# ferdean/lsa-fw

Measured on AMD Instinct MI355X. Metric: converged eigenpairs/sec (k=20, shift-invert), higher is better.
Workload: dtype c128

## Files before the change

### lsa-fw_amd/csrc/ndlu.hip

```cpp
#include "ndlu_internal.h"

namespace {

void nd_free(lsa_ndlu* f) {
    if (!f) return;
    ndlu_multi_free(f);
    for (void* p : {f->d_top, (void*)f->d_top_icmap, (void*)f->d_top_jobs, (void*)f->d_top_tiles})
        if (p) (void)hipFree(p);
    for (void* p : {(void*)f->d_lnodes_bwd, (void*)f->d_dist_nodes, (void*)f->d_child_ptr, (void*)f->d_child_idx, f->d_xstage, f->d_xg, (void*)f->d_tgoff, f->d_tg})
        if (p) (void)hipFree(p);
    for (void* p : {(void*)f->d_nodes, (void*)f->d_lnodes, (void*)f->d_gell, (void*)f->d_idx, (void*)f->d_cmap, (void*)f->d_tiles,
                    (void*)f->d_chunk_nodes, (void*)f->d_asm_dst, (void*)f->d_asm_src, (void*)f->d_ipiv, (void*)f->d_rowq, (void*)f->d_flag, (void*)f->d_xflag, (void*)f->d_maxabs,
                    f->d_lfac, f->d_ufac, f->d_work, f->d_upd, f->d_ubuf, f->d_xb, f->d_acc, f->d_tmp, f->d_ybuf, (void*)f->d_cand[0], (void*)f->d_cand[1], f->d_dinv})
        if (p) (void)hipFree(p);
    if (f->ev_panel) (void)hipEventDestroy(f->ev_panel);
    if (f->ev_pivots) (void)hipEventDestroy(f->ev_pivots);
    if (f->side) (void)hipStreamDestroy(f->side);
    delete f;
}

int nd_setup_top(lsa_ctx* ctx, lsa_ndlu* f, const std::vector<NdNodeDev>& nodes) {
    const NdSymbolic& S = f->S;
    f->top = NdTop{};
    f->top_level = -1;
// ... 56 lines not shown
    f->top_tiles[0] = (int32_t)tiles.size() / 2;
    for (int32_t ci = 0; ci < K; ++ci)
        for (int32_t di = 0; di < K; ++di) {
            const NdNodeDev &nc = nodes[(size_t)S.child_idx[(size_t)c0 + ci]], &nd = nodes[(size_t)S.child_idx[(size_t)c0 + di]];
            add(NdTopJob{tp.node[ci].off * s + oR, nd.lfac_off + (int64_t)nd.m * nd.m, tp.node[ci].off * s + tp.node[di].off, ci == di ? nc.lfac_off : -1, nc.m,
                         nd.m, nd.f - nd.m, (int32_t)s, nd.m, nc.m, 2, 1, nd.cmap_off, 0});
        }
    f->top_tiles[1] = (int32_t)tiles.size() / 2 - f->top_tiles[0];
    LSA_CHECK(upload(ctx, icmap, &f->d_top_icmap));
    LSA_CHECK(upload(ctx, jobs, &f->d_top_jobs));
    LSA_CHECK(upload(ctx, tiles, &f->d_top_tiles));
    LSA_HIP_ALLOC(ctx, hipMalloc(&f->d_top, (size_t)(s * s) * esize(f->dtype)));
    f->top = tp;
    f->top_level = lr;
    f->top_replaced_entries = replaced;
    f->solve_launches -= 2;
    return LSA_OK;
}


struct TileBuffer {
    std::vector<int32_t> tiles;
    void begin(TileList& tl) {
        tl.off = (int64_t)tiles.size() / 2;
        tl.count = 0;
    }
    void push(TileList& tl, int32_t a, int32_t b) {
        tiles.push_back(a);
        tiles.push_back(b);
        ++tl.count;
    }
};

void nd_setup_knobs(lsa_ndlu* f) {
    const char* e = getenv("LSA_ND_TP_MIN");
    f->tp_min = e && *e ? std::max(1, atoi(e)) : 512;
    const char* sbm = getenv("LSA_ND_SB_MIN");
    f->sb_min = std::max(f->tp_min, sbm && *sbm ? std::max(1, atoi(sbm)) : 1024);
    f->ycap = kNB;
    const char* sbc = getenv("LSA_ND_SB_COLS");
    f->sb_cols = sbc && *sbc ? std::min(1024, std::max(kGT, atoi(sbc) / kGT * kGT)) : kSB;
}

bool nd_setup_ordered(const NdSymbolic& S) {
    const bool dist = S.nranks > 1;
    bool ordered = true;
    for (size_t k = 0; k < S.perm.size() && ordered; ++k) ordered = S.perm[k] == (int32_t)k || dist;
    if (dist)
        for (int32_t t = 0; t < S.nt && ordered; ++t)
            for (int32_t r = 1; r < S.m[(size_t)t]; ++r)
                if (S.idx[(size_t)S.idx_off[(size_t)t] + r] != S.idx[(size_t)S.idx_off[(size_t)t]] + r) {
                    ordered = false;
                    break;
                }
    return ordered;
}

int64_t nd_setup_budget(const NdSymbolic& S, size_t es, int64_t free_agreed) {
    size_t free_b = 0, total_b = 0;
    if (hipMemGetInfo(&free_b, &total_b) != hipSuccess) free_b = (size_t)16 << 30;
    const int64_t after = (int64_t)free_b - S.factor_entries * (int64_t)es;
    int64_t budget = std::max<int64_t>(after / 4, (int64_t)256 << 20) / (int64_t)es;
    if (S.has_dist) budget = std::max<int64_t>((free_agreed > 0 ? free_agreed : (int64_t)free_b) / 6, (int64_t)256 << 20) / (int64_t)es;
    if (const char* e = getenv("LSA_ND_WORK_MB")) budget = std::max<int64_t>(atoll(e), 1) * (1 << 20) / (int64_t)es;
    return budget;
}

std::vector<NdNodeDev> nd_setup_nodes(const NdSymbolic& S, const NdMemoryPlan& P) {
    std::vector<NdNodeDev> nodes((size_t)S.nt);
    for (int32_t t = 0; t < S.nt; ++t) {
        NdNodeDev& nd = nodes[(size_t)t];
// ... 95 lines not shown
        for (int32_t rb = r0; rb < r1; rb += sh)
            for (int32_t cb = 0; cb < TN; cb += sw)
                for (int32_t r = rb; r < std::min(rb + sh, r1); ++r)
                    for (int32_t cc = cb; cc < std::min(cb + sw, TN); ++cc) seq[x].push_back((r << 16) | cc);
    }
    size_t pos[8] = {0, 0, 0, 0, 0, 0, 0, 0};
    for (int64_t left = (int64_t)TM * TN; left > 0; --left) {
        int x = (int)(tl.count % 8);
        for (int tries = 0; tries < 8 && pos[x] >= seq[x].size(); ++tries) x = (x + 1) % 8;
        tb.push(tl, t, seq[x][pos[x]++]);
    }
}

void nd_setup_chunk_tiles(const NdSymbolic& S, NdChunk& c, TileBuffer& tb) {
    auto node = [&](int32_t q) { return S.lvl_nodes[(size_t)c.node_begin + q]; };
    int32_t lvl_children = 0;
    for (int32_t q = 0; q < c.node_count; ++q) lvl_children = std::max(lvl_children, S.child_ptr[(size_t)node(q) + 1] - S.child_ptr[(size_t)node(q)]);
    c.ext.assign((size_t)lvl_children, TileList());
    for (int32_t r = 0; r < lvl_children; ++r) {
        tb.begin(c.ext[(size_t)r]);
        for (int32_t q = 0; q < c.node_count; ++q) {
            const int32_t t = node(q);
            if (S.child_ptr[(size_t)t] + r >= S.child_ptr[(size_t)t + 1]) continue;
            const int32_t ch = S.child_idx[(size_t)S.child_ptr[(size_t)t] + r];
            if (S.kind[(size_t)t] == 4 && S.kind[(size_t)ch] != 2) continue;
            const int32_t bc = S.f[(size_t)ch] - S.m[(size_t)ch];
            for (int32_t i0 = 0; i0 < bc; i0 += 16) tb.push(c.ext[(size_t)r], ch, i0);
        }
    }
    tb.begin(c.unperm);
    for (int32_t q = 0; q < c.node_count; ++q)
        for (int32_t r0 = 0; r0 < S.m[(size_t)node(q)]; r0 += 16) tb.push(c.unperm, node(q), r0);
    static const bool xcd_order = !(getenv("LSA_ND_XCD_ORDER") && atoi(getenv("LSA_ND_XCD_ORDER")) == 0);
    for (int kind = 0; kind < 3; ++kind) {
        tb.begin(c.gemm[kind]);
        for (int32_t q = 0; q < c.node_count; ++q) {
            const int32_t t = node(q);
            const int32_t m = S.m[(size_t)t], b = S.f[(size_t)t] - m;
            if (b == 0) continue;
            const int32_t M = kind == 2 ? S.orows[(size_t)t] : S.brow[(size_t)t], N = kind == 0 ? m : b;
            if (M == 0) continue;
            const int32_t TM = (M + kGT - 1) / kGT, TN = (N + kGT - 1) / kGT;
            if ((int64_t)TM * TN >= 512 && xcd_order) {
                nd_push_xcd_order(tb, c.gemm[kind], t, TM, TN);
                continue;
            }
            for (int32_t tm = 0; tm < TM; ++tm)
                for (int32_t tn = 0; tn < TN; ++tn) tb.push(c.gemm[kind], t, (tm << 16) | tn);
        }
    }
    tb.begin(c.save);
    for (int32_t q = 0; q < c.node_count; ++q) {
        const int32_t t = node(q);
        for (int32_t r0 = 0; r0 < S.brow[(size_t)t]; r0 += 16) tb.push(c.save, t, r0);
    }
}

void nd_setup_chunk_xsteps(const NdSymbolic& S, const NdMemoryPlan& P, NdChunk& c) {
    std::vector<std::vector<NdChunk::XPiece>> queue((size_t)S.nranks);
    for (int32_t q = 0; q < c.node_count; ++q) {
        const int32_t t = S.lvl_nodes[(size_t)c.node_begin + q];
        if (S.kind[(size_t)t] != 4) continue;
        for (int32_t cp = S.child_ptr[(size_t)t]; cp < S.child_ptr[(size_t)t + 1]; ++cp) {
            const int32_t ch = S.child_idx[(size_t)cp];
            if (S.kind[(size_t)ch] == 2) continue;
            const int32_t bc = S.f[(size_t)ch] - S.m[(size_t)ch];
            if (bc == 0) continue;
// ... 250 lines not shown
    if (!ctx || !f || !C) return lsa_set_error(ctx, LSA_ERR_ARG, "lsa_ndlu_refactor: null argument");
    if (C->n != f->S.n || C->n != C->ncols || C->nnz != f->S.nnz || C->dtype != f->dtype)
        return lsa_set_error(ctx, LSA_ERR_ARG, "lsa_ndlu_refactor: the matrix does not match the analysed pattern");
    const double t0 = now_s();
    const int rc = ndlu_numeric(ctx, f, C);
    f->seconds_numeric = now_s() - t0;
    return rc;
}

static uint64_t mat_pattern_hash(const lsa_mat* P) {
    if (!P->h_hash) P->h_hash = std::make_shared<uint64_t>(0);
    if (*P->h_hash == 0) {
        const uint64_t h = nd_pattern_hash(P->n, P->h_rp.data(), P->h_ci.data());
        *P->h_hash = h ? h : 1;
    }
    return *P->h_hash;
}

static int nd_symbolic_phase(lsa_ctx* ctx, const lsa_mat* P, int dtype, int32_t leaf_size, const int8_t* constraint, bool strict,
                             lsa_ndlu** out) {
    *out = nullptr;
    if (P->n != P->ncols || P->row0 != 0) return lsa_set_error(ctx, LSA_ERR_ARG, "lsa_ndlu: needs a square, unsharded matrix");
    if ((int64_t)P->h_rp.size() != (int64_t)P->n + 1) return lsa_set_error(ctx, LSA_ERR_ARG, "lsa_ndlu: the matrix has no host copy of its pattern");
    if (leaf_size <= 0) leaf_size = nd_default_leaf(P->n);
    const double t0 = now_s();
    if (ctx->nd_cache) {
        lsa_ndlu* c = ctx->nd_cache;
        const uint64_t want = strict && constraint ? nd_constraint_hash(P->n, constraint) : 0;
        if (c->S.n == P->n && c->S.nnz == P->nnz && c->dtype == dtype && c->S.nranks == 1 && (c->S.tree_hash != 0 || c->S.leaf_size == leaf_size) &&
            (!strict || c->S.constraint_hash == want) &&
            c->S.pattern_hash == mat_pattern_hash(P)) {
            ctx->nd_cache = nullptr;
            c->seconds_analyse = 0.0;
            *out = c;
            return LSA_OK;
        }
        lsa_ndlu_drop_cache(ctx);
    }
    return nd_new_analysed(ctx, dtype, "lsa_ndlu", t0, 0, out, [&](NdSymbolic* S, char* err, int errlen) {
        return nd_analyse(P->n, P->h_rp.data(), P->h_ci.data(), leaf_size, constraint, S, err, errlen);
    });
}

int lsa_ndlu_prepare(lsa_ctx* ctx, const lsa_mat* P, int dtype, int32_t leaf_size, const int8_t* constraint) {
    if (!ctx || !P || (dtype != LSA_F64 && dtype != LSA_C128)) return lsa_set_error(ctx, LSA_ERR_ARG, "lsa_ndlu_prepare: bad argument");
    lsa_ndlu* f = nullptr;
    LSA_CHECK(nd_symbolic_phase(ctx, P, dtype, leaf_size, constraint, true, &f));
    lsa_ndlu_drop_cache(ctx);
    ctx->nd_cache = f;
    return LSA_OK;
}

int lsa_ndlu_prepare_tree(lsa_ctx* ctx, const lsa_mat* P, int dtype, int32_t ntree, const int32_t* first, const int32_t* size, const int32_t* parent) {
    if (!ctx || !P || (dtype != LSA_F64 && dtype != LSA_C128) || ntree < 0 || (ntree > 0 && (!first || !size || !parent)))
        return lsa_set_error(ctx, LSA_ERR_ARG, "lsa_ndlu_prepare_tree: bad argument");
    if (P->n != P->ncols || P->row0 != 0) return lsa_set_error(ctx, LSA_ERR_ARG, "lsa_ndlu_prepare_tree: needs a square, unsharded matrix");
    if ((int64_t)P->h_rp.size() != (int64_t)P->n + 1) return lsa_set_error(ctx, LSA_ERR_ARG, "lsa_ndlu_prepare_tree: the matrix has no host copy of its pattern");
    const double t0 = now_s();
    lsa_ndlu_drop_cache(ctx);
    lsa_ndlu* f = nullptr;
    LSA_CHECK(nd_new_analysed(ctx, dtype, "lsa_ndlu_prepare_tree", t0, 0, &f, [&](NdSymbolic* S, char* err, int errlen) {
        return nd_analyse_tree(P->n, P->h_rp.data(), P->h_ci.data(), ntree, first, size, parent, nullptr, 0, 1, S, err, errlen);
    }));
    ctx->nd_cache = f;
    return LSA_OK;
}
// ... 24 lines not shown
        return rc;
    }
    *out = f;
    return LSA_OK;
}

int lsa_ndlu_create_tree(lsa_ctx* ctx, const lsa_mat* C, int32_t ntree, const int32_t* first, const int32_t* size, const int32_t* parent,
                         const int32_t* owner, lsa_ndlu** out) {
    if (!ctx || !C || !out || ntree < 0) return lsa_set_error(ctx, LSA_ERR_ARG, "lsa_ndlu_create_tree: bad argument");
    *out = nullptr;
    if (C->n != C->ncols || C->row0 != 0) return lsa_set_error(ctx, LSA_ERR_ARG, "lsa_ndlu_create_tree: needs the whole square matrix (every rank holds it)");
    if ((int64_t)C->h_rp.size() != (int64_t)C->n + 1) return lsa_set_error(ctx, LSA_ERR_ARG, "lsa_ndlu_create_tree: the matrix has no host copy of its pattern");
    const double t0 = now_s();
    lsa_ndlu* f = nullptr;
    int setup_rc = LSA_OK;
    int64_t free_agreed = 0;
    if (ctx->nranks > 1) {
        size_t free_b = 0, total_b = 0;
        if (hipMemGetInfo(&free_b, &total_b) != hipSuccess) free_b = (size_t)16 << 30;
        if (ctx->nd_cache) {
            const lsa_ndlu* c = ctx->nd_cache;
            free_b += (size_t)(c->lfac_entries + c->ufac_entries + c->work_entries + c->upd_entries) * esize(c->dtype);
        }
        free_agreed = (int64_t)free_b;
        LSA_CHECK(k_agree_min_i64(ctx, &free_agreed));
    }
    if (ctx->nd_cache) {
        lsa_ndlu* c = ctx->nd_cache;
        if (c->S.tree_hash == nd_tree_hash(ntree, first, size, parent, owner, ctx->rank, ctx->nranks) && c->S.n == C->n && c->S.nnz == C->nnz && c->dtype == C->dtype &&
            c->S.pattern_hash == mat_pattern_hash(C)) {
            f = c;
            ctx->nd_cache = nullptr;
            f->seconds_analyse = 0.0;
        } else {
            lsa_ndlu_drop_cache(ctx);
        }
    }
    if (!f)
        setup_rc = nd_new_analysed(ctx, C->dtype, "lsa_ndlu_create_tree", t0, free_agreed, &f, [&](NdSymbolic* S, char* err, int errlen) {
            return nd_analyse_tree(C->n, C->h_rp.data(), C->h_ci.data(), ntree, first, size, parent, owner, ctx->rank, ctx->nranks, S, err, errlen);
        });
    setup_rc = k_agree_status(ctx, setup_rc);
    if (setup_rc != LSA_OK) {
        nd_free(f);
        return setup_rc;
    }
    const int rc = lsa_ndlu_refactor(ctx, f, C);
    if (rc != LSA_OK) {
        nd_free(f);
        return rc;
    }
    *out = f;
    return LSA_OK;
}

void lsa_ndlu_destroy(lsa_ndlu* f) {
    if (!f) return;
    lsa_ctx* ctx = f->ctx;
    if (ctx && ctx->stream) (void)hipStreamSynchronize(ctx->stream);
    if (ctx && !getenv("LSA_ND_NO_CACHE")) {
        lsa_ndlu_drop_cache(ctx);
        ctx->nd_cache = f;
        return;
    }
    nd_free(f);
}
// ... 193 lines not shown
```

### lsa-fw_amd/csrc/ndlu_factor.hip

```cpp
#include "ndlu_internal.h"

namespace {

template <typename T>
__global__ __launch_bounds__(256) void nd_maxabs2_kernel(int64_t nnz, const T* __restrict__ v, unsigned long long* __restrict__ out) {
    __shared__ double wmax[4];
    double best = 0.0;
    const int64_t stride = (int64_t)gridDim.x * blockDim.x;
    for (int64_t i = (int64_t)blockIdx.x * blockDim.x + threadIdx.x; i < nnz; i += stride) {
        const double a = s_abs2(v[i]);
        if (a == a && a > best) best = a;
        else if (a != a) best = a;
    }
    for (int o = 32; o > 0; o >>= 1) {
        const double other = __shfl_xor(best, o);
        best = (best != best) ? best : (other != other) ? other : fmax(best, other);
    }
    if ((threadIdx.x & 63) == 0) wmax[threadIdx.x >> 6] = best;
    __syncthreads();
    if (threadIdx.x == 0) {
        for (int w = 1; w < 4; ++w) best = (best != best) ? best : (wmax[w] != wmax[w]) ? wmax[w] : fmax(best, wmax[w]);
        atomicMax(out, (unsigned long long)__double_as_longlong(best));
    }
}
// ... 308 lines not shown
        const int32_t gc = col0 + qb;
        Ys[jb][qb] = (jb < nb && gc < m) ? yb[(size_t)jb * m + gc] : scalar_traits<T>::zero();
    }
    __syncthreads();
    T acc[4][4];
#pragma unroll
    for (int i = 0; i < 4; ++i)
#pragma unroll
        for (int j = 0; j < 4; ++j) acc[i][j] = scalar_traits<T>::zero();
    for (int k = 0; k < nb; ++k) {
        T av[4], bv[4];
#pragma unroll
        for (int i = 0; i < 4; ++i) av[i] = Ws[k][ty * 4 + i];
#pragma unroll
        for (int j = 0; j < 4; ++j) bv[j] = Ys[k][tx + 16 * j];
#pragma unroll
        for (int i = 0; i < 4; ++i)
#pragma unroll
            for (int j = 0; j < 4; ++j) fma_acc(acc[i][j], av[i], bv[j]);
    }
#pragma unroll
    for (int i = 0; i < 4; ++i) {
        const int32_t gr = row0 + ty * 4 + i;
        if (gr >= m) continue;
        const int32_t q = rq[gr];
        const bool is_piv = q >= kb && q < kb + nb;
#pragma unroll
        for (int j = 0; j < 4; ++j) {
            const int32_t gc = col0 + tx + 16 * j;
            if (gc >= m || (gc >= kb && gc < kb + nb)) continue;
            if ((gc >= skip_lo && gc < skip_hi) || (only_hi > only_lo && (gc < only_lo || gc >= only_hi))) continue;
            T* cptr = a + (size_t)gr * ld + gc;
            *cptr = is_piv ? acc[i][j] : s_add(*cptr, acc[i][j]);
        }
    }
}

constexpr int kTA = 8;

template <typename T>
struct tp_first {
    static constexpr int RPT = sizeof(T) == 16 ? 1 : 2;
    static constexpr int rows = 256 * RPT;
};

__host__ __device__ inline int32_t tp_sets(int32_t m, int32_t first_rows, int32_t round) {
    int32_t n = (m + first_rows - 1) / first_rows;
    for (int32_t r = 0; r < round; ++r) n = (n + kTA - 1) / kTA;
    return n;
}

template <typename T, bool FIRST, bool LAST>
__global__ __launch_bounds__(256) void nd_tp_round_kernel(const int32_t* __restrict__ lvl_nodes, const NdNodeDev* __restrict__ nodes,
                                                          const T* __restrict__ front, int32_t* __restrict__ ipiv, int32_t* __restrict__ rowq, int32_t kb,
                                                          int32_t round, const int32_t* __restrict__ cand_in, int32_t* __restrict__ cand_out,
                                                          T* __restrict__ dinv, int32_t* __restrict__ flag, double tiny2) {
    constexpr int RPT = FIRST ? tp_first<T>::RPT : 1;
    __shared__ unsigned long long skey[2];
    __shared__ T prow_s[2][kNB];
    __shared__ int32_t sel_s[kNB];
    __shared__ T Ds[LAST ? kNB : 1][kNB + 1];
    const int32_t t = lvl_nodes[blockIdx.x];
    const NdNodeDev nd = nodes[t];
    const int32_t m = nd.m, ld = nd.f;
    const int32_t w = min(kNB, m - kb);
    if (w <= 0) return;
// ... 233 lines not shown
                sm.Bs[p][(e >> 6) * LDBS + (e & 63)] = plane_of(pb[s], p);
            }
        }
        __syncthreads();
        if (kk + BK < K) gload(kk + BK);
#pragma unroll
        for (int k4 = 0; k4 < BK; k4 += 4) {
            if (kk + k4 >= K) break;
            double a[NPL][2], bb[NPL][2];
#pragma unroll
            for (int p = 0; p < NPL; ++p)
#pragma unroll
                for (int i = 0; i < 2; ++i) {
                    a[p][i] = sm.As[p][(wr + 16 * i + l15) * LDAS + k4 + l4];
                    bb[p][i] = sm.Bs[p][(k4 + l4) * LDBS + wc + 16 * i + l15];
                }
#pragma unroll
            for (int i = 0; i < 2; ++i)
#pragma unroll
                for (int j = 0; j < 2; ++j) {
                    acc[0][i][j] = __builtin_amdgcn_mfma_f64_16x16x4f64(a[0][i], bb[0][j], acc[0][i][j], 0, 0, 0);
                    if constexpr (NPL == 2) {
                        acc[0][i][j] = __builtin_amdgcn_mfma_f64_16x16x4f64(-a[NPL - 1][i], bb[NPL - 1][j], acc[0][i][j], 0, 0, 0);
                        acc[NPL - 1][i][j] = __builtin_amdgcn_mfma_f64_16x16x4f64(a[0][i], bb[NPL - 1][j], acc[NPL - 1][i][j], 0, 0, 0);
                        acc[NPL - 1][i][j] = __builtin_amdgcn_mfma_f64_16x16x4f64(a[NPL - 1][i], bb[0][j], acc[NPL - 1][i][j], 0, 0, 0);
                    }
                }
        }
        __syncthreads();
    }
}

template <typename T, int KIND>
__global__ __launch_bounds__(256) void nd_gemm_mfma_kernel(const int32_t* __restrict__ tiles, const NdNodeDev* __restrict__ nodes,
                                                           T* __restrict__ front, T* __restrict__ lfac, T* __restrict__ ufac) {
    constexpr int NPL = MfmaTile<T>::NPL;
    __shared__ MfmaTile<T> sm;
    const int32_t t = tiles[2 * blockIdx.x], packed = tiles[2 * blockIdx.x + 1];
    const int32_t tm = packed >> 16, tn = packed & 0xFFFF;
    const NdNodeDev nd = nodes[t];
    const int32_t m = nd.m, f = nd.f, b = f - m;
    T* F = front + nd.front_off;
    T* inv = nd.inv_off < 0 ? lfac + nd.lfac_off : front + nd.inv_off;
    T* invrows = lfac + nd.lfac_off;
    T* S1 = invrows + (size_t)nd.orows * m;
    T* S2 = ufac + nd.ufac_off;
    const T *A, *B;
    T* C;
    int32_t M, N, K, lda, ldb, ldc;
    if (KIND == 0) {
        A = F + (size_t)m * f, lda = f, B = inv, ldb = m, C = S1, ldc = m, M = nd.brow, N = m, K = m;
    } else if (KIND == 1) {
        A = S1, lda = m, B = F + m, ldb = f, C = F + (size_t)m * f + m, ldc = f, M = nd.brow, N = b, K = m;
    } else {
        A = invrows, lda = m, B = F + m, ldb = f, C = S2, ldc = b, M = nd.orows, N = b, K = m;
    }
    const int32_t row0 = tm * kGT, col0 = tn * kGT;
    mfma_d4 acc[NPL][2][2];
    mfma_tile_product<T>(
        K,
        [&](int r, int32_t k) {
            const int32_t gr = row0 + r;
            return (gr < M && k < K) ? A[(size_t)gr * lda + k] : scalar_traits<T>::zero();
        },
        [&](int32_t k, int c) {
            const int32_t gc = col0 + c;
            return (k < K && gc < N) ? B[(size_t)k * ldb + gc] : scalar_traits<T>::zero();
        },
        sm, acc);
    const int lane = threadIdx.x & 63, wave = threadIdx.x >> 6;
    const int wr = 32 * (wave >> 1), wc = 32 * (wave & 1), l15 = lane & 15, l4 = lane >> 4;
#pragma unroll
    for (int i = 0; i < 2; ++i)
#pragma unroll
        for (int r = 0; r < 4; ++r) {
            const int32_t gr = row0 + wr + 16 * i + l4 + 4 * r;
            if (gr >= M) continue;
#pragma unroll
            for (int j = 0; j < 2; ++j) {
                const int32_t gc = col0 + wc + 16 * j + l15;
                if (gc >= N) continue;
                T v;
                s_from(v, acc[0][i][j][r], acc[NPL - 1][i][j][r]);
                T* c = C + (size_t)gr * ldc + gc;
                if (KIND == 0) *c = s_sub(scalar_traits<T>::zero(), v);
                else if (KIND == 1) *c = s_add(*c, v);
                else *c = v;
            }
        }
}

template <typename T>
__global__ __launch_bounds__(256) void nd_gj_update_kernel(const int32_t* __restrict__ lvl_nodes, const NdNodeDev* __restrict__ nodes,
                                                           T* __restrict__ front, const int32_t* rowq, int32_t kb, int32_t kw,
                                                           const T* __restrict__ ybuf, int32_t ycap, int32_t only_lo, int32_t only_hi,
                                                           int32_t skip_lo, int32_t skip_hi, int32_t ztile0) {
    constexpr int NPL = MfmaTile<T>::NPL;
    __shared__ MfmaTile<T> sm;
    const int32_t t = lvl_nodes[blockIdx.x];
    const NdNodeDev nd = nodes[t];
    const int32_t m = nd.m, ld = nd.f;
    const int32_t nb = min(kw, m - kb);
    const int32_t row0 = (int32_t)blockIdx.y * kGT, col0 = ((int32_t)blockIdx.z + ztile0) * kGT;
    if (nb <= 0 || row0 >= m || col0 >= m) return;
    if (col0 >= kb && col0 + kGT <= kb + nb) return;
    if (only_hi > only_lo && (col0 >= only_hi || col0 + kGT <= only_lo)) return;
    if (col0 >= skip_lo && col0 + kGT <= skip_hi) return;
    T* a = front + nd.front_off;
    const T* yb = ybuf + (size_t)ycap * nd.piv_off;
    const int32_t* rq = rowq + nd.piv_off;
    mfma_d4 acc[NPL][2][2];
    mfma_tile_product<T>(
        nb,
        [&](int r, int32_t k) {
            const int32_t gr = row0 + r;
            return (gr < m && k < nb) ? a[(size_t)gr * ld + kb + k] : scalar_traits<T>::zero();
        },
        [&](int32_t k, int c) {
            const int32_t gc = col0 + c;
            return (k < nb && gc < m) ? yb[(size_t)k * m + gc] : scalar_traits<T>::zero();
        },
        sm, acc);
// ... 69 lines not shown
#pragma unroll
        for (int g = 0; g < 2; ++g) {
            const int32_t i = i0 + ti + 16 * h, j = j0 + tj + 16 * g;
            if (i >= jb.M || j >= jb.N) continue;
            const T d = jb.d_off >= 0 ? lfac[jb.d_off + (size_t)i * jb.ldd + j] : scalar_traits<T>::zero();
            top[jb.c_off + (size_t)i * ldc + j] = jb.negate ? s_sub(d, acc[h][g]) : s_add(d, acc[h][g]);
        }
}

template <typename T, int NT, int RPT, int W>
void launch_block(lsa_ctx* ctx, lsa_ndlu* f, const NdChunk& L, int32_t kb, double tiny2) {
    hipStream_t st = ctx->stream;
    const int32_t* lv = f->d_chunk_nodes + L.node_begin;
    T* front = (T*)f->d_work;
    auto active_at = [&](int32_t k) {
        return (int32_t)(std::lower_bound(L.sorted_m.begin(), L.sorted_m.end(), k, std::greater<int32_t>()) - L.sorted_m.begin());
    };
    const int32_t kend = std::min(kb + kNB, L.max_m);
    const bool others = std::min(kNB, L.max_m - kb) > W;
    int32_t kprev = -1, active_prev = 0;
    for (int32_t k0 = kb; k0 < kend; k0 += W) {
        const int32_t active = active_at(k0);
        if (active == 0) break;
        hipLaunchKernelGGL((nd_gj_fused_kernel<T, NT, RPT, W>), dim3(std::max(active, active_prev), others && kprev >= 0 ? 1 + kNB / 16 : 1), dim3(NT), 0, st, lv,
                           f->d_nodes, front, f->d_ipiv, f->d_rowq, kb, k0, kprev, f->d_flag, tiny2);
        kprev = k0;
        active_prev = active;
    }
    if (others && kprev >= 0)
        hipLaunchKernelGGL((nd_gj_fused_kernel<T, NT, RPT, W>), dim3(active_prev, 1 + kNB / 16), dim3(NT), 0, st, lv, f->d_nodes, front, f->d_ipiv, f->d_rowq, kb,
                           -1, kprev, f->d_flag, tiny2);
    if (L.max_m > kNB) {
        const int32_t active = active_at(kb);
        hipLaunchKernelGGL((nd_gj_stage_kernel<T>), dim3(active, (L.max_m + 255) / 256), dim3(256), 0, st, lv, f->d_nodes, (const T*)front, f->d_ipiv, kb,
                           kNB, kNB, 0, L.max_m, (T*)f->d_ybuf);
        const int32_t tiles = (L.max_m + kGT - 1) / kGT;
        hipLaunchKernelGGL((nd_gj_gemm_kernel<T>), dim3(active, tiles, tiles), dim3(256), 0, st, lv, f->d_nodes, front, f->d_rowq, kb, (const T*)f->d_ybuf, 0, 0,
                           0, 0, 0);
    }
}

template <typename T>
void launch_tournament(lsa_ndlu* f, const NdChunk& L, int32_t kb, double tiny2, hipStream_t st) {
    const int32_t* lv = f->d_chunk_nodes + L.node_begin;
    const T* front = (const T*)f->d_work;
    const int32_t active = (int32_t)(std::lower_bound(L.sorted_m.begin(), L.sorted_m.end(), kb, std::greater<int32_t>()) - L.sorted_m.begin());
    if (active == 0) return;
    int32_t sets = (L.max_m + tp_first<T>::rows - 1) / tp_first<T>::rows;
    hipLaunchKernelGGL((nd_tp_round_kernel<T, true, false>), dim3(active, sets), dim3(256), 0, st, lv, f->d_nodes, front, f->d_ipiv, f->d_rowq, kb, 0,
                       (const int32_t*)nullptr, f->d_cand[0], (T*)nullptr, f->d_flag, tiny2);
    int src = 0;
    for (int32_t round = 0;; ++round) {
        const int32_t groups = (sets + kTA - 1) / kTA;
        if (groups == 1) {
            hipLaunchKernelGGL((nd_tp_round_kernel<T, false, true>), dim3(active, 1), dim3(256), 0, st, lv, f->d_nodes, front, f->d_ipiv, f->d_rowq, kb, round,
                               (const int32_t*)f->d_cand[src], (int32_t*)nullptr, (T*)f->d_dinv, f->d_flag, tiny2);
            break;
        }
        hipLaunchKernelGGL((nd_tp_round_kernel<T, false, false>), dim3(active, groups), dim3(256), 0, st, lv, f->d_nodes, front, f->d_ipiv, f->d_rowq, kb, round,
                           (const int32_t*)f->d_cand[src], f->d_cand[src ^ 1], (T*)nullptr, f->d_flag, tiny2);
        src ^= 1;
        sets = groups;
    }
}

template <typename T>
// ... 94 lines not shown
        LSA_HIP_CHECK(ctx, hipMemsetAsync(f->d_work, 0, (size_t)L.work_entries * sizeof(T), st));
        if (L.asm_count > 0) {
            const int blocks = (int)std::min<int64_t>((L.asm_count + 255) / 256, (int64_t)ctx->num_cu * 16);
            hipLaunchKernelGGL((nd_assemble_kernel<T>), dim3(blocks), dim3(256), 0, st, L.asm_count, (const T*)C->val, f->d_asm_src + L.asm_begin,
                               f->d_asm_dst + L.asm_begin, front);
        }
        for (const TileList& e : L.ext)
            if (e.count > 0)
                hipLaunchKernelGGL((nd_extend_add_kernel<T>), dim3(e.count), dim3(256), 0, st, tl + 2 * e.off, f->d_nodes, f->d_cmap, front, (const T*)upd);
        for (const auto& step : L.xsteps) {
            T* stage = (T*)f->d_xstage;
            int64_t stride = 0;
            for (int r = 0; r < S.nranks; ++r) {
                const NdChunk::XPiece& pc = step[(size_t)r];
                if (pc.nrows > 0) stride = std::max(stride, (int64_t)pc.nrows * (S.f[(size_t)pc.child] - S.m[(size_t)pc.child]));
            }
            if (stride == 0) continue;
            const NdChunk::XPiece& mine = step[(size_t)S.rank];
            if (mine.nrows > 0) {
                const int32_t bc = S.f[(size_t)mine.child] - S.m[(size_t)mine.child];
                const int64_t src_off = f->chunk_node_upd_off(mine.child) + (int64_t)(mine.row0 - S.brow0[(size_t)mine.child]) * bc;
                LSA_HIP_CHECK(ctx, hipMemcpyAsync(stage + (size_t)S.rank * (size_t)stride, upd + src_off, (size_t)mine.nrows * (size_t)bc * sizeof(T),
                                                  hipMemcpyDeviceToDevice, st));
            }
            LSA_CHECK(k_allgather_inplace(ctx, stage, (size_t)stride * sizeof(T)));
            for (int r = 0; r < S.nranks; ++r) {
                const NdChunk::XPiece& pc = step[(size_t)r];
                if (pc.nrows <= 0) continue;
                hipLaunchKernelGGL((nd_extend_add_staged_kernel<T>), dim3((pc.nrows + 15) / 16), dim3(256), 0, st, f->d_nodes, f->d_cmap, front,
                                   (const T*)(stage + (size_t)r * (size_t)stride), pc.child, pc.row0, pc.nrows);
            }
        }
        if (L.max_m >= f->tp_min) LSA_CHECK(launch_level_tp<T>(ctx, f, L, tiny2));
        for (int32_t kb = 0; kb < L.max_m && L.max_m < f->tp_min; kb += kNB) {
            if (L.max_m <= 64) launch_block<T, 64, 1, 8>(ctx, f, L, kb, tiny2);
            else if (L.max_m <= 128) launch_block<T, 128, 1, 8>(ctx, f, L, kb, tiny2);
            else if (L.max_m <= 256) launch_block<T, 256, 1, 8>(ctx, f, L, kb, tiny2);
            else if (L.max_m <= 512) launch_block<T, 512, 1, 8>(ctx, f, L, kb, tiny2);
            else if (L.max_m <= 1024) launch_block<T, 1024, 1, 8>(ctx, f, L, kb, tiny2);
            else if (L.max_m <= 2048) launch_block<T, 1024, 2, 8>(ctx, f, L, kb, tiny2);
            else if (L.max_m <= 4096) launch_block<T, 1024, 4, 4>(ctx, f, L, kb, tiny2);
            else if (L.max_m <= 8192) launch_block<T, 1024, 8, 2>(ctx, f, L, kb, tiny2);
            else launch_block<T, 1024, 16, 1>(ctx, f, L, kb, tiny2);
        }
        if (L.unperm.count > 0)
            hipLaunchKernelGGL((nd_unperm_kernel<T>), dim3(L.unperm.count), dim3(256), 0, st, tl + 2 * L.unperm.off, f->d_nodes, front, f->d_ipiv,
                               f->d_rowq, lfac);
        auto product = [&](auto kind) {
            constexpr int KIND = decltype(kind)::value;
            if (L.gemm[KIND].count == 0) return;
            hipLaunchKernelGGL((nd_gemm_mfma_kernel<T, KIND>), dim3(L.gemm[KIND].count), dim3(256), 0, st, tl + 2 * L.gemm[KIND].off, f->d_nodes, front, lfac, ufac);
        };
        product(std::integral_constant<int, 0>{});
        product(std::integral_constant<int, 1>{});
        product(std::integral_constant<int, 2>{});
        if (L.save.count > 0)
            hipLaunchKernelGGL((nd_save_update_kernel<T>), dim3(L.save.count), dim3(256), 0, st, tl + 2 * L.save.off, f->d_nodes, (const T*)front, upd);
    }
    if (f->top.s > 0)
        for (int q = 0, t0 = 0; q < 2; t0 += f->top_tiles[q++])
            if (f->top_tiles[q] > 0)
                hipLaunchKernelGGL((nd_top_gemm_kernel<T>), dim3(f->top_tiles[q]), dim3(256), 0, st, f->d_top_tiles + 2 * t0, f->d_top_jobs, f->d_cmap,
                                   (const T*)lfac, (const T*)ufac, (T*)f->d_top, f->top.s);
    if (!exchanged && S.nranks > 1 && f->xupd_slot > 0)
        LSA_CHECK(k_allgather_inplace(ctx, f->d_upd, (size_t)f->xupd_slot * sizeof(T)));
    int32_t hflag[4] = {0, 0, 0, 0};
    if (S.nranks > 1) {
        LSA_HIP_CHECK(ctx, hipMemcpyAsync(f->d_xflag + 4 * S.rank, f->d_flag, 4 * sizeof(int32_t), hipMemcpyDeviceToDevice, st));
        LSA_CHECK(k_allgather_inplace(ctx, f->d_xflag, 4 * sizeof(int32_t)));
        std::vector<int32_t> all((size_t)4 * S.nranks, 0);
        LSA_HIP_CHECK(ctx, hipMemcpyAsync(all.data(), f->d_xflag, all.size() * sizeof(int32_t), hipMemcpyDeviceToHost, st));
        LSA_HIP_CHECK(ctx, hipStreamSynchronize(st));
        for (int r = 0; r < S.nranks; ++r)
            if (all[(size_t)4 * r + 1] != 0) {
                memcpy(hflag, &all[(size_t)4 * r], sizeof hflag);
                if (r != S.rank) hflag[1] = -(r + 1);
                break;
            }
    } else {
        LSA_HIP_CHECK(ctx, hipMemcpyAsync(hflag, f->d_flag, sizeof hflag, hipMemcpyDeviceToHost, st));
        LSA_HIP_CHECK(ctx, hipStreamSynchronize(st));
    }
    LSA_HIP_CHECK(ctx, hipGetLastError());
    if (hflag[1] < 0)
        return lsa_set_error(ctx, LSA_ERR_ZERO_PIVOT, "lsa_ndlu: a pivot block on rank %d is singular to 1e-15 * max|C| (column %d of its node)", -hflag[1] - 1,
                             hflag[2]);
    if (hflag[1] != 0) {
        const int32_t t = hflag[1] - 1;
// ... 26 lines not shown
```

### lsa-fw_amd/csrc/ndlu_internal.h

```cpp
#pragma once
#include <algorithm>
#include <chrono>
#include <cmath>
#include <cstdlib>
#include <functional>
#include <new>
#include <string>

#include "lsa_internal.h"
#include "nd_internal.h"

int k_allgather_inplace(lsa_ctx* ctx, void* vec, size_t bytes_per_rank);

constexpr int kRT = 32;
constexpr int kSweepWide = 512;
constexpr int kCH = 1024;
constexpr int kGT = 64;
constexpr int kNB = 32;
constexpr int kSB = 128;
constexpr int kTRmin = 256;
constexpr int kNdBatchMax = 16;
static_assert(kNdBatchMax == kKrylovGroupMax, "a lockstep round hands all its problems to one batched sweep");
constexpr int kMCH = 256;
constexpr int kNdMultiMax = 8;
// ... 88 lines not shown
    NdSymbolic S;
    int dtype = LSA_C128;
    bool ordered = false;
    std::vector<NdChunk> chunks;
    std::vector<NdLevel> levels;
    NdNodeDev* d_nodes = nullptr;
    NdSweepNode *d_lnodes = nullptr, *d_lnodes_bwd = nullptr;
    int32_t *d_dist_nodes = nullptr, *d_child_ptr = nullptr, *d_child_idx = nullptr;
    void *d_xstage = nullptr, *d_xg = nullptr;
    int64_t* d_tgoff = nullptr;
    void* d_tg = nullptr;
    std::vector<int64_t> tg_slot;
    int64_t tg_slot_max = 0;
    int64_t xstage_slot = 0;
    std::vector<int64_t> h_upd_off, h_lfac_off;
    int64_t chunk_node_upd_off(int32_t t) const { return h_upd_off[(size_t)t]; }
    int32_t* d_gell = nullptr;
    int32_t *d_idx = nullptr, *d_cmap = nullptr, *d_tiles = nullptr, *d_chunk_nodes = nullptr;
    int64_t* d_asm_dst = nullptr;
    int32_t* d_asm_src = nullptr;
    int64_t asm_count = 0;
    int32_t *d_ipiv = nullptr, *d_rowq = nullptr, *d_flag = nullptr, *d_xflag = nullptr;
    unsigned long long* d_maxabs = nullptr;
    void *d_lfac = nullptr, *d_ufac = nullptr;
    void *d_work = nullptr, *d_upd = nullptr;
    void *d_ubuf = nullptr, *d_xb = nullptr, *d_acc = nullptr;
    void *d_tmp = nullptr, *d_ybuf = nullptr;
    int64_t lfac_entries = 0, ufac_entries = 0, work_entries = 0, upd_entries = 0, acc_entries = 0;
    int64_t xupd_slot = 0;
    int32_t *d_cand[2] = {nullptr, nullptr};
    void* d_dinv = nullptr;
    int32_t tp_min = 1 << 30;
    int32_t sb_min = 1 << 30;
    int32_t sb_cols = 128;
    int32_t ycap = 32;
    hipStream_t side = nullptr;
    hipEvent_t ev_panel = nullptr, ev_pivots = nullptr;
    double seconds_analyse = 0.0, seconds_numeric = 0.0;
    int32_t solve_launches = 0;
    NdTop top = {};
    int32_t top_level = -1;
    void* d_top = nullptr;
    int32_t* d_top_icmap = nullptr;
    NdTopJob* d_top_jobs = nullptr;
    int32_t* d_top_tiles = nullptr;
    int32_t top_tiles[2] = {0, 0};
    int64_t top_replaced_entries = 0;
    int acc_vbytes = 0;
    struct MultiColumn {
        void *ubuf = nullptr, *xb = nullptr, *acc = nullptr, *tmp = nullptr;
        int acc_vbytes = 0;
    };
    std::vector<MultiColumn> multi;
    bool multi_full = false;
    int64_t multi_bytes = 0;
    int32_t multi_width = 0;
    bool multi_transposed = false;
};

template <typename U>
int upload(lsa_ctx* ctx, const std::vector<U>& h, U** d) {
    const size_t bytes = std::max<size_t>(h.size(), 1) * sizeof(U);
    LSA_HIP_ALLOC(ctx, hipMalloc((void**)d, bytes));
    if (!h.empty()) LSA_HIP_CHECK(ctx, hipMemcpy(*d, h.data(), h.size() * sizeof(U), hipMemcpyHostToDevice));
    return LSA_OK;
}
// ... 7 lines not shown
```

Before: 588.7.

## Add register-resident blocked Gauss-Jordan panel kernel and fuse GEMM kinds 0 and 2

Adds a register-resident Gauss-Jordan kernel for fronts of up to 256 rows. Each thread holds one row's 32-column panel in registers and processes pivots in sub-panels of 8, with a shared-memory trailing update between them; this replaces the multi-launch panel factorization for small levels. It also reorders the GEMM tile lists so kinds 0 and 2 sit next to each other, letting one paired kernel launch cover both. The aim is fewer launches and less global-memory traffic per panel, at the cost of more register pressure and a new pivoting code path that can be turned off with an environment knob.

Measured after the change: 596.0, median of 4. No clear change (+1.2%).

```diff
diff --git a/lsa-fw_amd/csrc/ndlu.hip b/lsa-fw_amd/csrc/ndlu.hip
--- a/lsa-fw_amd/csrc/ndlu.hip
+++ b/lsa-fw_amd/csrc/ndlu.hip
@@ -112,11 +112,17 @@
     }
 };
 
+bool nd_knob_gj_block() {
+    const char* e = getenv("LSA_ND_GJ_BLOCK");
+    return !(e && *e && atoi(e) == 0);
+}
+
 void nd_setup_knobs(lsa_ndlu* f) {
     const char* e = getenv("LSA_ND_TP_MIN");
     f->tp_min = e && *e ? std::max(1, atoi(e)) : 512;
     const char* sbm = getenv("LSA_ND_SB_MIN");
     f->sb_min = std::max(f->tp_min, sbm && *sbm ? std::max(1, atoi(sbm)) : 1024);
+    f->gj_block = nd_knob_gj_block();
     f->ycap = kNB;
     const char* sbc = getenv("LSA_ND_SB_COLS");
     f->sb_cols = sbc && *sbc ? std::min(1024, std::max(kGT, atoi(sbc) / kGT * kGT)) : kSB;
@@ -278,7 +284,7 @@
     for (int32_t q = 0; q < c.node_count; ++q)
         for (int32_t r0 = 0; r0 < S.m[(size_t)node(q)]; r0 += 16) tb.push(c.unperm, node(q), r0);
     static const bool xcd_order = !(getenv("LSA_ND_XCD_ORDER") && atoi(getenv("LSA_ND_XCD_ORDER")) == 0);
-    for (int kind = 0; kind < 3; ++kind) {
+    for (int kind : {0, 2, 1}) {
         tb.begin(c.gemm[kind]);
         for (int32_t q = 0; q < c.node_count; ++q) {
             const int32_t t = node(q);
@@ -595,6 +601,7 @@
             c->S.pattern_hash == mat_pattern_hash(P)) {
             ctx->nd_cache = nullptr;
             c->seconds_analyse = 0.0;
+            c->gj_block = nd_knob_gj_block();
             *out = c;
             return LSA_OK;
         }
@@ -685,6 +692,7 @@
             f = c;
             ctx->nd_cache = nullptr;
             f->seconds_analyse = 0.0;
+            f->gj_block = nd_knob_gj_block();
         } else {
             lsa_ndlu_drop_cache(ctx);
         }
diff --git a/lsa-fw_amd/csrc/ndlu_factor.hip b/lsa-fw_amd/csrc/ndlu_factor.hip
--- a/lsa-fw_amd/csrc/ndlu_factor.hip
+++ b/lsa-fw_amd/csrc/ndlu_factor.hip
@@ -364,6 +364,135 @@
             if ((gc >= skip_lo && gc < skip_hi) || (only_hi > only_lo && (gc < only_lo || gc >= only_hi))) continue;
             T* cptr = a + (size_t)gr * ld + gc;
             *cptr = is_piv ? acc[i][j] : s_add(*cptr, acc[i][j]);
+        }
+    }
+}
+
+__device__ __forceinline__ double pick(bool k, double a, double b) { return k ? a : b; }
+__device__ __forceinline__ cplx pick(bool k, cplx a, cplx b) { return cplx{k ? a.re : b.re, k ? a.im : b.im}; }
+
+template <typename T, int NT>
+__global__ __launch_bounds__(NT) void nd_gj_block_kernel(const int32_t* __restrict__ lvl_nodes, const NdNodeDev* __restrict__ nodes,
+                                                         T* __restrict__ front, int32_t* __restrict__ ipiv, int32_t* __restrict__ rowq,
+                                                         int32_t kb, int32_t* __restrict__ flag, double tiny2) {
+    constexpr int W = 8;
+    __shared__ unsigned long long skey[kNB];
+    __shared__ T prow_s[2][W];
+    __shared__ int32_t prows[W];
+    __shared__ T ys[W][kNB];
+    const int32_t t = lvl_nodes[blockIdx.x];
+    const NdNodeDev nd = nodes[t];
+    const int32_t m = nd.m, ld = nd.f;
+    const int32_t nb = min(kNB, m - kb);
+    if (nb <= 0) return;
+    T* a = front + nd.front_off;
+    const int tid = threadIdx.x, lane = tid & 63;
+    int32_t* piv = ipiv + nd.piv_off;
+    int32_t* rq = rowq + nd.piv_off;
+    const bool row = tid < m;
+    T* ai = a + (size_t)min(tid, m - 1) * ld + kb;
+    if (tid < kNB) skey[tid] = 0ull;
+    bool used = !row || rq[min(tid, m - 1)] >= 0;
+    T r[kNB];
+#pragma unroll
+    for (int c = 0; c < kNB; ++c) {
+        const T v = ai[min(c, nb - 1)];
+        r[c] = (row && c < nb) ? v : scalar_traits<T>::zero();
+    }
+    __syncthreads();
+    int rot = 0;
+#pragma unroll 1
+    for (int pn = 0; pn < kNB / W; ++pn) {
+        const int32_t k0 = kb + W * pn;
+        const int32_t w = min(W, m - k0);
+        if (w <= 0) break;
+#pragma unroll 1
+        for (int jj = 0; jj < w; ++jj) {
+            unsigned long long key = used ? 0ull : pivot_key(s_abs2(r[0]), tid);
+            key = wave_max_key(key);
+            if (lane == 0) atomicMax(&skey[W * pn + jj], key);
+            __syncthreads();
+            key = skey[W * pn + jj];
+            const int32_t p = 65535 - (int32_t)(key & 0xFFFFull);
+            if (tid == 0) {
+                piv[k0 + jj] = p;
+                prows[jj] = p;
+                if (!(__longlong_as_double((long long)(key & ~0xFFFFull)) > tiny2) && atomicCAS(&flag[1], 0, t + 1) == 0) {
+                    flag[2] = k0 + jj;
+                    flag[3] = (int32_t)(key >> 32);
+                }
+            }
+            if (tid == p) {
+                T pv = r[0];
+                if (s_abs2(pv) == 0.0) s_from(pv, 1.0, 0.0);
+                const T pinv = s_inv(pv);
+#pragma unroll
+                for (int q = 0; q < W; ++q) {
+                    const T v = (q == 0) ? pinv : s_mul(pinv, r[q]);
+                    prow_s[jj & 1][q] = v;
+                    r[q] = v;
+                }
+                used = true;
+                rq[p] = k0 + jj;
+            }
+            __syncthreads();
+            if (row && tid != p) {
+                const T fm = r[0];
+                if (s_abs2(fm) != 0.0) {
+                    const T nfm = s_sub(scalar_traits<T>::zero(), fm);
+                    r[0] = scalar_traits<T>::zero();
+#pragma unroll
+                    for (int q = 0; q < W; ++q) fma_acc(r[q], nfm, prow_s[jj & 1][q]);
+                }
+            }
+            const T head = r[0];
+#pragma unroll
+            for (int q = 0; q + 1 < W; ++q) r[q] = r[q + 1];
+            r[W - 1] = head;
+        }
+#pragma unroll 1
+        for (int x = w; x < W; ++x) {
+            const T head = r[0];
+#pragma unroll
+            for (int q = 0; q + 1 < W; ++q) r[q] = r[q + 1];
+            r[W - 1] = head;
+        }
+        if (nb <= W) break;
+        int myj = -1;
+#pragma unroll
+        for (int j = 0; j < W; ++j)
+            if (j < w && prows[j] == tid) myj = j;
+        if (myj >= 0) {
+#pragma unroll
+            for (int q = 0; q < kNB; ++q) ys[myj][q] = r[q];
+        }
+        __syncthreads();
+#pragma unroll
+        for (int j = 0; j < W; ++j) r[j] = pick(j < w, r[j], scalar_traits<T>::zero());
+#pragma unroll
+        for (int q = W; q < kNB; ++q) {
+            T acc = myj >= 0 ? scalar_traits<T>::zero() : r[q];
+#pragma unroll
+            for (int j = 0; j < W; ++j) fma_acc(acc, r[j], j < w ? ys[j][q] : scalar_traits<T>::zero());
+            r[q] = pick(((q + W * pn) & (kNB - 1)) < nb, acc, r[q]);
+            __builtin_amdgcn_sched_barrier(0);
+        }
+#pragma unroll
+        for (int q = 0; q < W; ++q) {
+            const T keep = r[q];
+            r[q] = r[q + W];
+            r[q + W] = r[q + 2 * W];
+            r[q + 2 * W] = r[q + 3 * W];
+            r[q + 3 * W] = keep;
+        }
+        ++rot;
+    }
+    static_assert(kNB == 4 * W, "four panels per block");
+    if (row) {
+#pragma unroll
+        for (int q = 0; q < kNB; ++q) {
+            const int32_t c = (q + W * rot) & (kNB - 1);
+            if (c < nb) ai[c] = r[q];
         }
     }
 }
@@ -663,10 +792,9 @@
 }
 
 template <typename T, int KIND>
-__global__ __launch_bounds__(256) void nd_gemm_mfma_kernel(const int32_t* __restrict__ tiles, const NdNodeDev* __restrict__ nodes,
-                                                           T* __restrict__ front, T* __restrict__ lfac, T* __restrict__ ufac) {
+__device__ __forceinline__ void nd_gemm_mfma_tile(const int32_t* __restrict__ tiles, const NdNodeDev* __restrict__ nodes, T* __restrict__ front,
+                                                  T* __restrict__ lfac, T* __restrict__ ufac, MfmaTile<T>& sm) {
     constexpr int NPL = MfmaTile<T>::NPL;
-    __shared__ MfmaTile<T> sm;
     const int32_t t = tiles[2 * blockIdx.x], packed = tiles[2 * blockIdx.x + 1];
     const int32_t tm = packed >> 16, tn = packed & 0xFFFF;
     const NdNodeDev nd = nodes[t];
@@ -719,6 +847,21 @@
                 else *c = v;
             }
         }
+}
+
+template <typename T, int KIND>
+__global__ __launch_bounds__(256) void nd_gemm_mfma_kernel(const int32_t* __restrict__ tiles, const NdNodeDev* __restrict__ nodes,
+                                                           T* __restrict__ front, T* __restrict__ lfac, T* __restrict__ ufac) {
+    __shared__ MfmaTile<T> sm;
+    nd_gemm_mfma_tile<T, KIND>(tiles, nodes, front, lfac, ufac, sm);
+}
+
+template <typename T>
+__global__ __launch_bounds__(256) void nd_gemm_mfma_pair_kernel(const int32_t* __restrict__ tiles, int32_t n0, const NdNodeDev* __restrict__ nodes,
+                                                                T* __restrict__ front, T* __restrict__ lfac, T* __restrict__ ufac) {
+    __shared__ MfmaTile<T> sm;
+    if ((int32_t)blockIdx.x < n0) nd_gemm_mfma_tile<T, 0>(tiles, nodes, front, lfac, ufac, sm);
+    else nd_gemm_mfma_tile<T, 2>(tiles, nodes, front, lfac, ufac, sm);
 }
 
 template <typename T>
@@ -854,6 +997,23 @@
                            -1, kprev, f->d_flag, tiny2);
     if (L.max_m > kNB) {
         const int32_t active = active_at(kb);
+        hipLaunchKernelGGL((nd_gj_stage_kernel<T>), dim3(active, (L.max_m + 255) / 256), dim3(256), 0, st, lv, f->d_nodes, (const T*)front, f->d_ipiv, kb,
+                           kNB, kNB, 0, L.max_m, (T*)f->d_ybuf);
+        const int32_t tiles = (L.max_m + kGT - 1) / kGT;
+        hipLaunchKernelGGL((nd_gj_gemm_kernel<T>), dim3(active, tiles, tiles), dim3(256), 0, st, lv, f->d_nodes, front, f->d_rowq, kb, (const T*)f->d_ybuf, 0, 0,
+                           0, 0, 0);
+    }
+}
+
+template <typename T, int NT>
+void launch_block_one(lsa_ctx* ctx, lsa_ndlu* f, const NdChunk& L, int32_t kb, double tiny2) {
+    hipStream_t st = ctx->stream;
+    const int32_t* lv = f->d_chunk_nodes + L.node_begin;
+    T* front = (T*)f->d_work;
+    const int32_t active = (int32_t)(std::lower_bound(L.sorted_m.begin(), L.sorted_m.end(), kb, std::greater<int32_t>()) - L.sorted_m.begin());
+    if (active == 0) return;
+    hipLaunchKernelGGL((nd_gj_block_kernel<T, NT>), dim3(active), dim3(NT), 0, st, lv, f->d_nodes, front, f->d_ipiv, f->d_rowq, kb, f->d_flag, tiny2);
+    if (L.max_m > kNB) {
         hipLaunchKernelGGL((nd_gj_stage_kernel<T>), dim3(active, (L.max_m + 255) / 256), dim3(256), 0, st, lv, f->d_nodes, (const T*)front, f->d_ipiv, kb,
                            kNB, kNB, 0, L.max_m, (T*)f->d_ybuf);
         const int32_t tiles = (L.max_m + kGT - 1) / kGT;
@@ -1014,8 +1174,12 @@
             }
         }
         if (L.max_m >= f->tp_min) LSA_CHECK(launch_level_tp<T>(ctx, f, L, tiny2));
+        const bool one = f->gj_block && L.max_m <= 256;
         for (int32_t kb = 0; kb < L.max_m && L.max_m < f->tp_min; kb += kNB) {
-            if (L.max_m <= 64) launch_block<T, 64, 1, 8>(ctx, f, L, kb, tiny2);
+            if (one && L.max_m <= 64) launch_block_one<T, 64>(ctx, f, L, kb, tiny2);
+            else if (one && L.max_m <= 128) launch_block_one<T, 128>(ctx, f, L, kb, tiny2);
+            else if (one) launch_block_one<T, 256>(ctx, f, L, kb, tiny2);
+            else if (L.max_m <= 64) launch_block<T, 64, 1, 8>(ctx, f, L, kb, tiny2);
             else if (L.max_m <= 128) launch_block<T, 128, 1, 8>(ctx, f, L, kb, tiny2);
             else if (L.max_m <= 256) launch_block<T, 256, 1, 8>(ctx, f, L, kb, tiny2);
             else if (L.max_m <= 512) launch_block<T, 512, 1, 8>(ctx, f, L, kb, tiny2);
@@ -1033,9 +1197,16 @@
             if (L.gemm[KIND].count == 0) return;
             hipLaunchKernelGGL((nd_gemm_mfma_kernel<T, KIND>), dim3(L.gemm[KIND].count), dim3(256), 0, st, tl + 2 * L.gemm[KIND].off, f->d_nodes, front, lfac, ufac);
         };
-        product(std::integral_constant<int, 0>{});
-        product(std::integral_constant<int, 1>{});
-        product(std::integral_constant<int, 2>{});
+        if (f->gj_block && L.gemm[0].count > 0 && L.gemm[2].count > 0 &&
+            L.gemm[2].off == L.gemm[0].off + L.gemm[0].count) {
+            hipLaunchKernelGGL((nd_gemm_mfma_pair_kernel<T>), dim3(L.gemm[0].count + L.gemm[2].count), dim3(256), 0, st, tl + 2 * L.gemm[0].off,
+                               L.gemm[0].count, f->d_nodes, front, lfac, ufac);
+            product(std::integral_constant<int, 1>{});
+        } else {
+            product(std::integral_constant<int, 0>{});
+            product(std::integral_constant<int, 1>{});
+            product(std::integral_constant<int, 2>{});
+        }
         if (L.save.count > 0)
             hipLaunchKernelGGL((nd_save_update_kernel<T>), dim3(L.save.count), dim3(256), 0, st, tl + 2 * L.save.off, f->d_nodes, (const T*)front, upd);
     }
diff --git a/lsa-fw_amd/csrc/ndlu_internal.h b/lsa-fw_amd/csrc/ndlu_internal.h
--- a/lsa-fw_amd/csrc/ndlu_internal.h
+++ b/lsa-fw_amd/csrc/ndlu_internal.h
@@ -144,6 +144,7 @@
     void* d_dinv = nullptr;
     int32_t tp_min = 1 << 30;
     int32_t sb_min = 1 << 30;
+    bool gj_block = true;
     int32_t sb_cols = 128;
     int32_t ycap = 32;
     hipStream_t side = nullptr;
```
